# kxhit/semantic-icp

Hardware: AMD Instinct MI355X
Metric: correspondences/sec (higher is better)
Workload: dtype f64

## Files before the change

### semantic-icp_amd/csrc/engine.hpp

```cpp
#ifndef SICP_ENGINE_HPP_
#define SICP_ENGINE_HPP_

#include <hip/hip_runtime.h>

#include <algorithm>
#include <array>
#include <atomic>
#include <chrono>
#include <condition_variable>
#include <cmath>
#include <cstdio>
#include <cstdlib>
#include <cstring>
#include <deque>
#include <limits>
#include <memory>
#include <mutex>
#include <new>
#include <string>
#include <thread>
#include <unordered_map>
#include <unordered_set>
#include <vector>

// ... 249 lines not shown
  DevBuf<double> proj;
  bool proj_valid = false;
  DevBuf<int> nn;
  int nn_stride = 0;
  bool feat_valid = false;
  int feat_k = 0, feat_C = 0, feat_float_products = 0;
  bool feat_hist = false;
  unsigned long long feat_epoch = 0;
  unsigned long long proj_cm_id = 0;
  OwnedEvent ready_ev;
  std::atomic<bool> pending{false};
  int n_seg() const { return (int)seg_label.size(); }
  int caller_index(int d) const { return keep.empty() ? perm[d] : keep[perm[d]]; }
};

constexpr int kPoolDevices = 64;
constexpr size_t kPoolCap = 1024;
struct CloudPool {
  std::mutex m;
  std::vector<Cloud*> free_list[kPoolDevices];
};
CloudPool& cloud_pool();
std::shared_ptr<Cloud> acquire_cloud(int device);
unsigned long long next_epoch();
double now_ms();
bool debug_enabled();

struct JobSlice {
  int knn_K = 0;
  std::vector<sicp::KnnArgs> knn;
  std::vector<sicp::CovArgs> cov;
  std::vector<sicp::ProjArgs> proj;
  std::vector<sicp::WeightArgs> weight;
  std::vector<sicp::CountJob> count;
  struct Sizes { size_t knn = 0, cov = 0, proj = 0, weight = 0, count = 0; };
  Sizes sizes() const { return {knn.size(), cov.size(), proj.size(), weight.size(), count.size()}; }
  void shrink_to(const Sizes& s) { knn.resize(s.knn); cov.resize(s.cov); proj.resize(s.proj); weight.resize(s.weight); count.resize(s.count); }
  void clear() { shrink_to(Sizes()); }
  bool empty() const { return knn.empty() && cov.empty() && proj.empty() && weight.empty() && count.empty(); }
};

constexpr int kParts = 4;

struct JobCollector {
  bool fold_weights = false;
  int slice = 0;
  JobSlice part[kParts];
};

struct TickSet {
  DevBuf<sicp::BatchArgs> d_batch;
  DevBuf<sicp::BatchHeader> d_bhdr;
  HostBuf<sicp::BatchHeader> h_bhdr;
  HostBuf<sicp::BatchArgs> h_batch;
  HostBuf<sicp::LmJoin> h_join;
  DevBuf<sicp::LmJoin> d_join;
  int cap = 0;
  sicp::BatchGraph graph[2];
  bool static_ranges = false;
  std::vector<int> tick_act;
  bool tick_valid = false;
  TickSet() = default;
  TickSet(const TickSet&) = delete;
  TickSet& operator=(const TickSet&) = delete;
  ~TickSet() { sicp::batch_graph_destroy(graph[0]); sicp::batch_graph_destroy(graph[1]); }
  void invalidate() { tick_valid = false; tick_act.clear(); static_ranges = false; }
};

}
}

using namespace sicp::host;

struct sicp_use_state {
  JobCollector* collect = nullptr;
  sicp_params params;
  unsigned long long epoch = 0;
  int C = 0;
  std::vector<double> cm;
  unsigned long long cm_id = 0;
  int corr_n = 0, corr_K = 0;
  bool corr_valid = false, corr_weighted = false;
  bool hint_ok = false;
  int solo_pair = 0;
  bool solo_was_init = false, solo_failed = false;
  int solo_skip = 0, solo_penalty = 0;
  bool count_stats = false;
  bool counted_in_search = false;
  bool wait_on_device = false;
  std::string last_error;
  sicp_stats st = {};
  sicp_use_state() { sicp_default_params(SICP_MODE_GICP, &params); }
};

struct sicp_context : sicp_use_state {
  int device = 0;
  bool parked = false;
  std::shared_ptr<Cloud> cl[2];
  Cloud& cloud(int which) { return *cl[which]; }
  const Cloud& cloud(int which) const { return *cl[which]; }
  OwnedStream own_stream, own_stream2;
  OwnedStream side_stream;
  OwnedStream feat_stream;
  OwnedStream part_stream[kParts];
  JobSlice own_jobs;
  hipStream_t stream = nullptr, stream2 = nullptr;
  OwnedEvent ev0, ev1, ev_join;
  OwnedEvent side_done, side_done2, main_done;
  std::vector<OwnedEvent> chunk_ev;
  OwnedEvent part_fork, part_done[kParts];
  DevBuf<double> d_cm, d_hval;
  int hval_k = 0;
  DevBuf<int> idx;
  DevBuf<float> d2;
  DevBuf<double> w;
  DevBuf<unsigned long long> part;
  DevBuf<double> partials, out28;
  DevBuf<long long> d_count;
  DevBuf<sicp::LmState> d_lm;
  HostBuf<sicp::LmState> h_lm;
  HostBuf<double> h_out28;
  HostBuf<long long> h_count;
  DevBuf<float> tmpx, tmpy, tmpz;
  DevBuf<double> tmp9;
  DevBuf<uint32_t> tmpl;
  HostBuf<uint32_t> h_labels;
  HostBuf<unsigned char> pc_stage;
  DevBuf<int> ev_idx;
  DevBuf<float> ev_d2;
  HostBuf<unsigned char> ev_stage;
  HostBuf<unsigned char> mg_stage;
  HostBuf<uint32_t> mg_out;
  TickSet ts[2];
  DevBuf<sicp::LmState> d_bstates;
  DevBuf<double> d_bout28;
  HostBuf<sicp::LmState> h_bstates{hipHostMallocCoherent};
  HostBuf<double> h_bout28;
  DevBuf<unsigned> d_solo_sync;
  unsigned solo_tag = 0;
  int solo_seq = 0;
  HostBuf<int> h_solo_flag{hipHostMallocCoherent};

  void reset_use() {
    static_cast<sicp_use_state&>(*this) = sicp_use_state();
    stream = own_stream;
    stream2 = own_stream2;
    for (TickSet& S : ts) S.invalidate();
  }
};

struct StreamCloudRef;
namespace sicp {
namespace host {
struct PoseCovSums {
  double out28[28];
  double sums[42];
  long long active;
};
struct PoseCovStream;
}
}
struct sicp_stream_ctx {
  int device = 0, cap = 0;
  sicp_params params;
  int C = 0;
  std::vector<double> cm;
// ... 426 lines not shown
```

### semantic-icp_amd/csrc/kernels.h

```cpp
#ifndef SICP_KERNELS_H_
#define SICP_KERNELS_H_

#include <hip/hip_runtime.h>
#include <stdint.h>

#include "bvh.hpp"
#include "lm.hpp"

#ifndef SICP_HD
#define SICP_HD
#endif

namespace sicp {

struct Pose {
  double R[9];
  double t[3];
};

struct Mat4f {
  float m[16];
};

struct alignas(16) PointRec {
// ... 3 lines not shown
  float z;
  uint32_t pad_[3];
};
static_assert(sizeof(PointRec) == 48, "PointRec is read with three dwordx4 / dwordx2 loads");

#ifndef SICP_SG4
#define SICP_SG4 4
#endif
#ifndef SICP_ACC_OCC
#define SICP_ACC_OCC 2
#endif
constexpr int acc_slots_per_group(int K) { return K % 4 == 0 ? SICP_SG4 : 2; }

struct AccGeometry {
  int n_groups, steps, chunk_groups, n_chunks;
};
SICP_HD inline AccGeometry acc_geometry(int total_slots, int slots_per_group) {
  AccGeometry g;
  const int per_lane = 8 / slots_per_group;
  g.n_groups = (total_slots + slots_per_group - 1) / slots_per_group;
  int m = (g.n_groups + 256 * per_lane * 1024 - 1) / (256 * per_lane * 1024);
  if (m < 1) m = 1;
  g.steps = per_lane * m;
  g.chunk_groups = 256 * g.steps;
  g.n_chunks = (g.n_groups + g.chunk_groups - 1) / g.chunk_groups;
  if (g.n_chunks < 1) g.n_chunks = 1;
  return g;
}

struct LossArgs {
  double cauchy_a;
  int use_sqloss;
};

struct NNArgs {
  const float *qx, *qy, *qz;
  int q_begin, q_count;
  int do_xform;
  double M[12];
  const float4* pts4;
  int t_begin, t_count;
  int chunk_len;
  unsigned long long* part;
};

struct MergeArgs {
  int q_begin, q_count, n_chunks;
  const unsigned long long* part;
  const int* inv;
  float gate_sq;
  int* out_i;
  float* out_d;
  int k_out;
};

struct TreeArgs {
  const float4* pts4;
  const float4* box_lo;
  const float4* box_hi;
  const unsigned long long* leaf_code;
  TreeLevels lv;
  int n;
  int pt_begin;
  int node_begin;
  int code_begin;
  float lo[3];
  float scale;
};

struct KnnArgs {
  const float *qx, *qy, *qz;
  int q_begin, q_count;
  int do_xform;
  double M[12];
  TreeArgs tree;
  int self;
  float gate_sq;
  const int* inv;
  int* out_i;
  float* out_d;
  int* dbg;
  const int* seed_hint;
  int hint_K, t_begin;
  int out_stride;
  int k_out;
  unsigned long long* live_cnt;
  const PointRec *w_srec, *w_trec;
  const double *w_sproj, *w_tproj;
  double* w_out;
  double w_one_m_eps;
  int w_C, w_bool_probability;
};
constexpr int kLiveCounters = 1024;

struct CovArgs {
  int n, k, C;
  const float *x, *y, *z;
  const uint32_t* label;
  const int* nn;
  int nn_stride;
  int float_products;
  PointRec* rec;
  uint8_t* hist;
  char* rec_dense;
  int rec_dense_n;
};

SICP_HD inline size_t dense_rec_bytes(int n) { return (size_t)(n > 0 ? n : 1) * 36; }
constexpr int kDenseGatherMaxPoints = 1 << 27;

SICP_HD inline int hist_stride(int C) { return (C + 15) & ~15; }

SICP_HD inline int proj_stride(int C) { return (C + 1) & ~1; }

struct ProjArgs {
  int n, C;
  const uint8_t* hist;
  const double* cm;
  const double* hval;
  double* proj;
};

struct WeightArgs {
  int n_s, K, C;
  const int* idx;
  const PointRec *srec, *trec;
  const double *s_proj, *t_proj;
  const uint8_t *s_hist, *t_hist;
  const double *cm, *hval;
  Pose pose;
  double one_m_eps;
  int bool_probability;
  double* w;
};

struct AccArgs {
  int n_s, K;
  const int* idx;
  const double* w;
  const PointRec *srec, *trec;
  const char* srec_dense;
  const char* trec_dense;
  int n_t, pad_;
  Pose pose;
  const LmState* lm;
  LmState* lm_step;
  double one_m_eps;
  LossArgs loss;
  double* partials;
};

struct GenAccArgs {
  AccArgs a;
  const double *scov6, *tcov6;
  int n_chunks, pad_;
};
hipError_t launch_accumulate_general(const GenAccArgs& g, hipStream_t st);

constexpr int kMaxKnnJobs = 8;
constexpr int kMaxSmallJobs = 16;
struct KnnJobs { KnnArgs job[kMaxKnnJobs]; };
struct CovJobs { CovArgs job[kMaxSmallJobs]; };
struct ProjJobs { ProjArgs job[kMaxSmallJobs]; };
struct WeightJobs { WeightArgs job[kMaxKnnJobs]; };
struct CountJob { const int* idx; int n; unsigned long long* out; };
struct CountJobs { CountJob job[kMaxSmallJobs]; };
// ... 480 lines not shown
```

### semantic-icp_amd/csrc/knn_kernels.hip

```cpp
#include <hip/hip_runtime.h>
#include <stdint.h>
#include <stdlib.h>

#define SICP_HD __host__ __device__
#include "kernels.h"
#include "device_geometry.hpp"

namespace sicp {

__device__ __forceinline__ float xform_row(const double* m, double x, double y, double z) {
#pragma clang fp contract(off)
  double a = __dmul_rn(m[0], x);
  a = __dadd_rn(a, __dmul_rn(m[1], y));
  a = __dadd_rn(a, __dmul_rn(m[2], z));
  a = __dadd_rn(a, m[3]);
  return __double2float_rn(a);
}

__device__ __forceinline__ float l2_simple(float ax, float ay, float az, float bx, float by, float bz) {
#pragma clang fp contract(off)
  const float dx = __fsub_rn(ax, bx), dy = __fsub_rn(ay, by), dz = __fsub_rn(az, bz);
  float r = __fmul_rn(dx, dx);
  r = __fadd_rn(r, __fmul_rn(dy, dy));
  r = __fadd_rn(r, __fmul_rn(dz, dz));
// ... 181 lines not shown
}

template <int K, int Q, int BS, int TILE>
__global__ __launch_bounds__(BS) void nn_partial_kernel(NNArgs a) {
  __shared__ float4 tile[TILE];
  const int chunk = blockIdx.y;
  const int c_lo = chunk * a.chunk_len;
  const int c_hi = min(c_lo + a.chunk_len, a.t_count);

  float px[Q], py[Q], pz[Q], wd[Q];
  u64 bk[Q][K];
#pragma unroll
  for (int j = 0; j < Q; ++j) {
    int q = blockIdx.x * (BS * Q) + j * BS + threadIdx.x;
    q = min(q, a.q_count - 1);
    load_query(a.qx, a.qy, a.qz, a.q_begin + q, a.do_xform, a.M, px[j], py[j], pz[j]);
#pragma unroll
    for (int k = 0; k < K; ++k) bk[j][k] = KEY_EMPTY;
    wd[j] = key_dist(KEY_EMPTY);
  }

  for (int t0 = c_lo; t0 < c_hi; t0 += TILE) {
    const int n = min(TILE, c_hi - t0);
    __syncthreads();
    for (int p = threadIdx.x; p < n; p += BS) tile[p] = a.pts4[a.t_begin + t0 + p];
    __syncthreads();
#pragma unroll 4
    for (int p = 0; p < n; ++p) {
      const float4 t = tile[p];
#pragma unroll
      for (int j = 0; j < Q; ++j) consider<K>(bk[j], wd[j], l2_simple(px[j], py[j], pz[j], t.x, t.y, t.z), __float_as_uint(t.w));
    }
  }

#pragma unroll
  for (int j = 0; j < Q; ++j) {
    const int q = blockIdx.x * (BS * Q) + j * BS + threadIdx.x;
    if (q < a.q_count) {
      const size_t o = ((size_t)chunk * a.q_count + q) * K;
#pragma unroll
      for (int k = 0; k < K; ++k) a.part[o + k] = bk[j][k];
    }
  }
}

template <int K>
__global__ __launch_bounds__(256) void nn_merge_kernel(MergeArgs a) {
  const int q = blockIdx.x * blockDim.x + threadIdx.x;
  if (q >= a.q_count) return;
  u64 bk[K];
#pragma unroll
  for (int k = 0; k < K; ++k) bk[k] = KEY_EMPTY;
  for (int c = 0; c < a.n_chunks; ++c) {
    const size_t o = ((size_t)c * a.q_count + q) * K;
#pragma unroll
    for (int k = 0; k < K; ++k) {
      const u64 key = a.part[o + k];
      if (key < bk[K - 1]) key_insert<K>(bk, key);
    }
  }
  emit<K>(bk, a.inv, a.gate_sq, a.out_i, a.out_d, (size_t)(a.q_begin + q) * a.k_out, a.k_out);
}

__device__ __forceinline__ float box_lb(const float4 lo, const float4 hi, float px, float py, float pz) {
  const float ex = fmaxf(fmaxf(lo.x - px, px - hi.x), 0.f);
  const float ey = fmaxf(fmaxf(lo.y - py, py - hi.y), 0.f);
  const float ez = fmaxf(fmaxf(lo.z - pz, pz - hi.z), 0.f);
  return (ex * ex + ey * ey) + ez * ez;
}

__device__ __forceinline__ unsigned quad_min_u(unsigned v) {
  v = min(v, (unsigned)__builtin_amdgcn_mov_dpp((int)v, 0xB1, 0xf, 0xf, true));
  return min(v, (unsigned)__builtin_amdgcn_mov_dpp((int)v, 0x4E, 0xf, 0xf, true));
}
__device__ __forceinline__ unsigned quad_max_u(unsigned v) {
  v = max(v, (unsigned)__builtin_amdgcn_mov_dpp((int)v, 0xB1, 0xf, 0xf, true));
  return max(v, (unsigned)__builtin_amdgcn_mov_dpp((int)v, 0x4E, 0xf, 0xf, true));
}
template <int K>
__device__ __forceinline__ float quad_bound(const u64 (&bk)[K]) {
  constexpr int M = (K + 3) / 4;
  return __uint_as_float(min(quad_min_u((unsigned)(bk[K - 1] >> 32)), quad_max_u((unsigned)(bk[M - 1] >> 32))));
}

__device__ __forceinline__ void scan_points_quad4(const float4 (&t)[4], float px, float py, float pz, u64 (&bk)[4], float& wd) {
  u64 c[4];
  const knn_v2f qxy = {px, py};
#pragma unroll
  for (int p = 0; p < 4; ++p) c[p] = make_key(l2_simple_pk(qxy, pz, t[p].x, t[p].y, t[p].z), __float_as_uint(t[p].w));
  key_cswap(c[0], c[1]); key_cswap(c[2], c[3]); key_cswap(c[0], c[2]); key_cswap(c[1], c[3]); key_cswap(c[1], c[2]);
  double l[4];
#pragma unroll
  for (int i = 0; i < 4; ++i) {
    const double a = __longlong_as_double((long long)bk[i]), b = __longlong_as_double((long long)c[3 - i]);
    asm("v_min_f64 %0, %1, %2" : "=v"(l[i]) : "v"(a), "v"(b));
  }
#pragma unroll
  for (int i = 0; i < 4; ++i) bk[i] = (u64)__double_as_longlong(l[i]);
  key_cswap(bk[0], bk[2]); key_cswap(bk[1], bk[3]); key_cswap(bk[0], bk[1]); key_cswap(bk[2], bk[3]);
  wd = quad_bound<4>(bk);
}

template <int K>
__device__ __forceinline__ void scan_points_quad(const float4 (&t)[4], float px, float py, float pz, u64 (&bk)[K], float& wd) {
  if constexpr (K == 4) { scan_points_quad4(t, px, py, pz, bk, wd); return; }
  if constexpr (K >= 8) {
    u64 c[4];
    const knn_v2f qxy = {px, py};
#pragma unroll
    for (int p = 0; p < 4; ++p) c[p] = make_key(l2_simple_pk(qxy, pz, t[p].x, t[p].y, t[p].z), __float_as_uint(t[p].w));
    key_cswap(c[0], c[1]); key_cswap(c[2], c[3]); key_cswap(c[0], c[2]); key_cswap(c[1], c[3]); key_cswap(c[1], c[2]);
#pragma unroll
    for (int r = 0; r < 4; ++r) {
      const bool pass = !(key_dist(c[r]) > wd) && c[r] < bk[K - 1];
      if (__ballot(pass) == 0) break;
      if (pass) key_insert<K>(bk, c[r]);
    }
  } else {
#pragma unroll
    for (int p = 0; p < 4; ++p) {
      const float d = l2_simple(px, py, pz, t[p].x, t[p].y, t[p].z);
      if (!(d > wd)) {
        const u64 key = make_key(d, __float_as_uint(t[p].w));
        if (key < bk[K - 1]) key_insert<K>(bk, key);
      }
    }
  }
  wd = quad_bound<K>(bk);
}

template <int K>
__device__ __forceinline__ void scan_leaf_quad(const float4* __restrict__ pts, float px, float py, float pz, u64 (&bk)[K], float& wd) {
  float4 t[4];
#pragma unroll
  for (int p = 0; p < 4; ++p) t[p] = pts[4 * p];
  scan_points_quad<K>(t, px, py, pz, bk, wd);
}

__device__ __forceinline__ unsigned child_mask_quad(const float4* __restrict__ blo, const float4* __restrict__ bhi, int child_off,
                                                    int child_cnt, int parent, int sub, int lane, float px, float py, float pz,
                                                    float wd) {
  const int c = parent * kFan + sub;
  const int node = child_off + min(c, child_cnt - 1);
  const float lb = box_lb(blo[node], bhi[node], px, py, pz);
  const bool ok = c < child_cnt && !(lb > wd);
  return (unsigned)(__ballot(ok) >> (lane & ~3)) & 15u;
}

template <int K>
__global__ __launch_bounds__(64) void bvh_knn_quad_kernel(KnnArgs a) {
  __shared__ int s_off[kMaxLevels], s_cnt[kMaxLevels];
  __shared__ u64 s_merge[16][4][K];
  if (threadIdx.x < kMaxLevels) { s_off[threadIdx.x] = a.tree.lv.off[threadIdx.x]; s_cnt[threadIdx.x] = a.tree.lv.cnt[threadIdx.x]; }
  __syncthreads();
  const int lane = threadIdx.x, sub = lane & 3, slot = lane >> 2;
  const int q_raw = blockIdx.x * 16 + slot;
  const int q = min(q_raw, a.q_count - 1);
  float px, py, pz;
  load_query(a.qx, a.qy, a.qz, a.q_begin + q, a.do_xform, a.M, px, py, pz);
  u64 bk[K];
  key_list_init<K>(bk);
  float wd = INFINITY;
  const float4* __restrict__ pts_all = a.tree.pts4 + a.tree.pt_begin;
  const float4* __restrict__ pts = pts_all + sub;
  const float4* __restrict__ blo = a.tree.box_lo + a.tree.node_begin;
  const float4* __restrict__ bhi = a.tree.box_hi + a.tree.node_begin;
  const int top = a.tree.lv.n_levels - 1;
  const int n_leaf = s_cnt[0];

  int seed = 0;
  if (top >= 1) {
    if (a.self) {
      seed = (q / kLeaf) / kFan;
    } else {
      const u64 qc = curve_code(px, py, pz, a.tree.lo[0], a.tree.lo[1], a.tree.lo[2], a.tree.scale);
      const u64* __restrict__ codes = a.tree.leaf_code + a.tree.code_begin;
      int lo_i = 0, hi_i = n_leaf - 1;
      while (lo_i < hi_i) {
        const int mid = (lo_i + hi_i + 1) >> 1;
        if (codes[mid] <= qc) lo_i = mid; else hi_i = mid - 1;
      }
      seed = lo_i / kFan;
    }
    const int l0 = seed * kFan, l1 = min(l0 + kFan, n_leaf);
    for (int l = l0; l < l1; ++l) scan_leaf_quad<K>(pts + (size_t)l * kLeaf, px, py, pz, bk, wd);
  } else {
    scan_leaf_quad<K>(pts, px, py, pz, bk, wd);
  }

  if (top >= 2) {
    unsigned masks = 0, masks_hi = 0;
    auto get = [&](int lv) -> unsigned { return lv < 8 ? (masks >> (4 * lv)) & 15u : (masks_hi >> (4 * (lv - 8))) & 15u; };
    auto put = [&](int lv, unsigned m) {
      if (lv < 8) masks = (masks & ~(15u << (4 * lv))) | (m << (4 * lv));
      else masks_hi = (masks_hi & ~(15u << (4 * (lv - 8)))) | (m << (4 * (lv - 8)));
    };
    int L = top - 1, base = 0;
    put(L, child_mask_quad(blo, bhi, s_off[L], s_cnt[L], 0, sub, lane, px, py, pz, wd));
    bool done = false;
    while (!done) {
      int leaf = -1;
      while (leaf < 0 && !done) {
        const unsigned m = get(L);
        if (m == 0) {
          if (L == top - 1) { done = true; break; }
          ++L;
          base = (base / kFan) & ~(kFan - 1);
          continue;
        }
        const int c = __ffs(m) - 1;
        put(L, m & (m - 1));
        const int node = base + c;
        if (L == 1 && node == seed) continue;
        if (L == 0) {
          leaf = node;
        } else {
          put(L - 1, child_mask_quad(blo, bhi, s_off[L - 1], s_cnt[L - 1], node, sub, lane, px, py, pz, wd));
          --L;
          base = node * kFan;
// ... 22 lines not shown
      const float d = best == KEY_EMPTY ? INFINITY : key_dist(best);
      const bool keep = orig != 0xffffffffu && d < a.gate_sq;
      a.out_i[o + k] = keep ? a.inv[orig] : -1;
      if (a.out_d) a.out_d[o + k] = d;
    }
  }
}

__device__ __forceinline__ int xcd_contiguous_block(int bid, int nblk) {
  const int q = nblk >> 3, r = nblk & 7;
  const int xcd = bid & 7, loc = bid >> 3;
  return xcd < r ? xcd * (q + 1) + loc : r * (q + 1) + (xcd - r) * q + loc;
}

__device__ __forceinline__ unsigned child_mask_packet(const float4* __restrict__ blo, const float4* __restrict__ bhi, int child_off,
                                                      int parent, int sub, float px, float py, float pz, float wd, float& lb) {
  const int node = child_off + parent * kFan + sub;
  lb = box_lb(blo[node], bhi[node], px, py, pz);
  const bool ok = !(lb > wd);
  u64 b = __ballot(ok);
  b |= b >> 32; b |= b >> 16; b |= b >> 8; b |= b >> 4;
  return (unsigned)b & 15u;
}

__device__ __forceinline__ int locate_leaf(const u64* __restrict__ codes, int top, u64 qc, int lane) {
  int lo = 0, shift = 2 * top;
  const int i = lane & 15;
  while (shift > 0) {
    const int s = shift >= 4 ? shift - 4 : 0;
    const bool probe = i >= 1 && i < (1 << (shift - s));
    const u64 c = probe ? codes[lo + (i << s)] : ~0ull;
    const u64 below = __ballot(probe && c <= qc) & 0xfffeull;
    lo += __popcll(below) << s;
    shift = s;
  }
  return lo;
}

constexpr int kWalkLevels = kMaxLevels - 1;

#ifndef SICP_KNN_DMA_MAXK
#define SICP_KNN_DMA_MAXK 4
#endif
#define KNN_LDS __attribute__((address_space(3)))
#define KNN_GLOBAL __attribute__((address_space(1)))
typedef float knn_v4f __attribute__((ext_vector_type(4)));
__device__ __forceinline__ void dma_leaf_group(const float4* __restrict__ pts_all, unsigned group, KNN_LDS knn_v4f* buf, int lane) {
  const float4* p = pts_all + (size_t)group * (kFan * kLeaf) + lane;
  __builtin_amdgcn_global_load_lds((const KNN_GLOBAL void*)p, (KNN_LDS void*)buf, 16, 0, 0);
}
__device__ __forceinline__ void lds_leaf_points(const KNN_LDS knn_v4f* buf, unsigned c, int sub, float4 (&t)[4]) {
#pragma unroll
  for (int p = 0; p < 4; ++p) {
    const knn_v4f v = buf[c * kLeaf + sub + 4 * p];
    t[p] = make_float4(v.x, v.y, v.z, v.w);
  }
}

template <int K, int WPB, bool LITERAL = false>
__device__ __forceinline__ void knn_packet_body(const KnnArgs& a, int wg, int n_wg) {
  constexpr size_t kWaveBytes = sizeof(float) * kWalkLevels * 64;
  __shared__ __attribute__((aligned(16))) unsigned char s_wave_all[WPB][kWaveBytes];
  constexpr bool kDma = K <= SICP_KNN_DMA_MAXK;
  __shared__ __attribute__((aligned(16))) float4 s_pts_all[kDma ? WPB : 1][kDma ? kFan * kLeaf : 1];
  KNN_LDS knn_v4f* const s_pts = (KNN_LDS knn_v4f*)s_pts_all[kDma ? (threadIdx.x >> 6) : 0];
  float (&s_lb)[kWalkLevels][64] = *reinterpret_cast<float (*)[kWalkLevels][64]>(s_wave_all[threadIdx.x >> 6]);
  const int lane = threadIdx.x & 63, sub = lane & 3, slot = lane >> 2;
  const int bid = xcd_contiguous_block(wg, n_wg) * WPB + (int)(threadIdx.x >> 6);
  if (bid * 16 >= a.q_count) return;
  const int q_raw = bid * 16 + slot;
  const int q = min(q_raw, a.q_count - 1);
  float px, py, pz;
  load_query(a.qx, a.qy, a.qz, a.q_begin + q, a.do_xform, a.M, px, py, pz);
  u64 bk[K];
  key_list_init<K>(bk);
  float wd = INFINITY;
  const float4* __restrict__ pts_all = a.tree.pts4 + a.tree.pt_begin;
  const float4* __restrict__ pts = pts_all + sub;
  const float4* __restrict__ blo = a.tree.box_lo + a.tree.node_begin;
  const float4* __restrict__ bhi = a.tree.box_hi + a.tree.node_begin;
  const int top = a.tree.lv.n_levels - 1;

  int n_box = 0, n_scan = 0;
  if (top == 0) {
    scan_leaf_quad<K>(pts, px, py, pz, bk, wd);
    ++n_scan;
  } else {
    int seed_leaf;
    if (a.self) {
      seed_leaf = bid;
    } else {
      int prev = -1;
      if (a.seed_hint) prev = __builtin_amdgcn_readlane(a.seed_hint[(size_t)(a.q_begin + q) * a.hint_K], 32);
      if (prev >= a.t_begin && prev < a.t_begin + a.tree.n) {
        seed_leaf = (prev - a.t_begin) / kLeaf;
      } else {
        const u64 qc_lane = curve_code_coarse<10>(px, py, pz, a.tree.lo[0], a.tree.lo[1], a.tree.lo[2], a.tree.scale);
        const u64 qc = ((u64)(unsigned)__builtin_amdgcn_readlane((int)(qc_lane >> 32), 32) << 32) |
                       (unsigned)__builtin_amdgcn_readlane((int)qc_lane, 32);
        seed_leaf = locate_leaf(a.tree.leaf_code + a.tree.code_begin, top, qc, lane);
      }
    }
    seed_leaf = __builtin_amdgcn_readfirstlane(seed_leaf);
    u64 masks = 0;
    float cur_lb = 0.f;
    constexpr int PB = 4;
    if constexpr (kDma) dma_leaf_group(pts_all, (unsigned)seed_leaf >> 2, s_pts, lane);
    for (int L0 = 0; L0 < top; L0 += PB) {
      float4 lo[PB], hi[PB];
#pragma unroll
      for (int i = 0; i < PB; ++i) {
        const int L = min(L0 + i, top - 1);
        const int node = level_offset(top, L) + (((seed_leaf >> (2 * L)) & ~3) + sub);
        lo[i] = blo[node];
        hi[i] = bhi[node];
      }
#pragma unroll
      for (int i = 0; i < PB; ++i) {
        const int L = L0 + i;
        if (L < top) {
          const float lb = box_lb(lo[i], hi[i], px, py, pz);
          s_lb[L][lane] = lb;
          if (L == 0) cur_lb = lb;
          u64 b = __ballot(lb < INFINITY);
          b |= b >> 32; b |= b >> 16; b |= b >> 8; b |= b >> 4;
          const unsigned m4 = ((unsigned)b & 15u) & ~(1u << ((seed_leaf >> (2 * L)) & 3));
          masks |= (u64)m4 << (4 * L);
          ++n_box;
        }
      }
    }
    if constexpr (K >= 16) {
      if constexpr (kDma) asm volatile("s_waitcnt vmcnt(0)" ::: "memory");
#pragma unroll
      for (int l = 0; l < kFan; ++l) {
        float4 t[4];
        if constexpr (kDma) {
          lds_leaf_points(s_pts, (unsigned)l, sub, t);
        } else {
#pragma unroll
          for (int p = 0; p < 4; ++p) t[p] = pts[(size_t)((seed_leaf & ~3) + l) * kLeaf + 4 * p];
        }
#pragma unroll
        for (int p = 0; p < 4; ++p) bk[4 * l + p] = make_key(l2_simple_pk(knn_v2f{px, py}, pz, t[p].x, t[p].y, t[p].z), __float_as_uint(t[p].w));
      }
      key_sort16<K>(bk);
      wd = quad_bound<K>(bk);
      masks &= ~15ull;
      n_scan += 4;
    } else {
      if constexpr (kDma) {
        asm volatile("s_waitcnt vmcnt(0)" ::: "memory");
        float4 t[4];
        lds_leaf_points(s_pts, (unsigned)seed_leaf & 3u, sub, t);
        scan_points_quad<K>(t, px, py, pz, bk, wd);
      } else {
        scan_leaf_quad<K>(pts + (size_t)seed_leaf * kLeaf, px, py, pz, bk, wd);
      }
      ++n_scan;
    }
    unsigned sh = 0u, ubase = (unsigned)seed_leaf & ~3u;
    const unsigned t4 = 1u << (2 * (top + 1));
    auto drop_unneeded = [&]() {
      u64 b = __ballot(!(cur_lb > wd));
      b |= b >> 32; b |= b >> 16; b |= b >> 8; b |= b >> 4;
      masks &= ~((u64)(~(unsigned)b & 15u) << sh);
    };
    drop_unneeded();
    for (;;) {
      int leaf = -1;
      for (;;) {
        const u64 rest = masks >> sh;
        if (rest == 0) break;
        const unsigned m = (unsigned)rest & 15u;
        if (m == 0) {
          const unsigned up = (unsigned)__builtin_ctzll(rest) & ~3u;
          sh += up;
          ubase = (ubase >> (up >> 1)) & ~3u;
          cur_lb = s_lb[sh >> 2][lane];
          drop_unneeded();
          continue;
        }
        const unsigned c = (unsigned)__ffs(m) - 1u;
        masks ^= 1ull << (sh + c);
        const unsigned node = ubase + c;
        if (sh == 0u) { leaf = (int)node; break; }
        ++n_box;
        sh -= 4u;
        ubase = node * kFan;
        if constexpr (kDma)
          if (sh == 0u) dma_leaf_group(pts_all, node, s_pts, lane);
        const unsigned cm = child_mask_packet(blo, bhi, (int)((t4 - (t4 >> (sh >> 1))) / 3u), (int)node, sub, px, py, pz, wd, cur_lb);
        masks |= (u64)cm << sh;
        s_lb[sh >> 2][lane] = cur_lb;
      }
      if (leaf < 0) break;
      if constexpr (kDma) {
        asm volatile("s_waitcnt vmcnt(0)" ::: "memory");
        float4 t[4];
        lds_leaf_points(s_pts, (unsigned)leaf & 3u, sub, t);
        scan_points_quad<K>(t, px, py, pz, bk, wd);
      } else {
        scan_leaf_quad<K>(pts + (size_t)leaf * kLeaf, px, py, pz, bk, wd);
      }
      ++n_scan;
      drop_unneeded();
    }
  }
  if (a.dbg && sub == 0 && q_raw < a.q_count) { a.dbg[2 * q] = n_box; a.dbg[2 * q + 1] = n_scan; }

  quad_merge<K>(bk);
  {
    const size_t o = a.out_stride > 0 ? (size_t)(a.q_begin + q) : (size_t)(a.q_begin + q) * a.k_out;
    const size_t ks = a.out_stride > 0 ? (size_t)a.out_stride : 1;
    unsigned live = 0;
#pragma unroll
    for (int t = 0; t < (K + 3) / 4; ++t) {
      u64 best = bk[4 * t < K ? 4 * t : K - 1];
#pragma unroll
      for (int s2 = 1; s2 < 4; ++s2)
        if (4 * t + s2 < K) best = sub == s2 ? bk[4 * t + s2] : best;
      const int k = 4 * t + sub;
      const bool mine = q_raw < a.q_count && k < K && k < a.k_out;
      const unsigned orig = (unsigned)best;
      const float d = best == KEY_EMPTY ? INFINITY : key_dist(best);
      const bool keep = orig != 0xffffffffu && d < a.gate_sq;
      int nb = -1;
      if (mine) {
        if (keep) nb = a.inv[orig];
        a.out_i[o + k * ks] = nb;
        if (a.out_d) a.out_d[o + k * ks] = d;
      }
      if (a.live_cnt) live += (unsigned)__popcll(__ballot(mine && keep));
      if constexpr (K == 4) {
        if (a.w_out != nullptr) {
          double w = 0.0;
          if (mine && nb >= 0) {
            const int C = a.w_C, PS = proj_stride(C), NP = PS / 2;
            typedef double v2d_t __attribute__((ext_vector_type(2)));
            const v2d_t* __restrict__ psrc = reinterpret_cast<const v2d_t*>(a.w_sproj + (size_t)(a.q_begin + q) * PS);
            const v2d_t* __restrict__ ptgt = reinterpret_cast<const v2d_t*>(a.w_tproj + (size_t)nb * PS);
            const PointRec sr = a.w_srec[a.q_begin + q], tr = a.w_trec[nb];
            double prob = 0.0;
            for (int kk = 0; kk < NP; ++kk) {
              const v2d_t tv = ptgt[kk], sv = psrc[kk];
              { double temp = tv.x; temp *= sv.x; prob += temp; }
              if (2 * kk + 1 < C) { double temp = tv.y; temp *= sv.y; prob += temp; }
            }
            Pose P;
#pragma unroll
            for (int r = 0; r < 3; ++r) {
              P.R[3 * r + 0] = a.M[4 * r + 0]; P.R[3 * r + 1] = a.M[4 * r + 1]; P.R[3 * r + 2] = a.M[4 * r + 2];
              P.t[r] = a.M[4 * r + 3];
            }
            w = prob * slot_gate<LITERAL>(P, a.w_one_m_eps, sr, tr, a.w_bool_probability);
          }
          if (mine) a.w_out[o + k * ks] = w;
        }
      }
    }
    if (a.live_cnt && lane == 0 && live) atomicAdd(a.live_cnt + (bid & (kLiveCounters - 1)), (unsigned long long)live);
  }
}

template <int K, int WPB, bool LITERAL = false>
__global__ __launch_bounds__(64 * WPB) void bvh_knn_packet_kernel(KnnArgs a) {
  knn_packet_body<K, WPB, LITERAL>(a, (int)blockIdx.x, (int)gridDim.x);
}

#ifndef SICP_KNN20_WAVES
#define SICP_KNN20_WAVES 1
#endif
template <int K, int WPB, bool LITERAL = false>
__global__ __launch_bounds__(64 * WPB, (K >= 16 ? SICP_KNN20_WAVES : 1)) void bvh_knn_packet_jobs_kernel(KnnJobs jobs) {
  const KnnArgs& a = jobs.job[blockIdx.y];
  const int n_wg = ((a.q_count + 15) / 16 + WPB - 1) / WPB;
  if ((int)blockIdx.x >= n_wg) return;
  knn_packet_body<K, WPB, LITERAL>(a, (int)blockIdx.x, n_wg);
}


static constexpr int NN_BS = 256;
static constexpr int NN_TILE = 1024;

int nn_queries_per_thread(int K) { return K == 1 ? 4 : (K <= 4 ? 2 : 1); }

// ... 86 lines not shown
```

### semantic-icp_amd/csrc/stages.cpp

```cpp
#include "engine.hpp"

namespace sicp {
namespace host {

static int launch_slice(sicp_context* h, JobSlice& s, hipStream_t st) {
  if (!s.knn.empty()) HIPCHECK(sicp::launch_bvh_knn_packet_jobs(s.knn_K, s.knn.data(), (int)s.knn.size(), st));
  if (!s.cov.empty()) HIPCHECK(sicp::launch_cov_jobs(s.cov.data(), (int)s.cov.size(), st));
  if (!s.proj.empty()) HIPCHECK(sicp::launch_proj_jobs(s.proj.data(), (int)s.proj.size(), st));
  if (!s.weight.empty()) HIPCHECK(sicp::launch_em_weight_jobs(s.weight.data(), (int)s.weight.size(), st));
  if (!s.count.empty()) HIPCHECK(sicp::launch_count_active_jobs(s.count.data(), (int)s.count.size(), st));
  s.clear();
  return SICP_OK;
}

struct OwnLaunch {
  bool launched = false;
  double ms = 0.0;
};
template <class Add>
static int hand_off(sicp_context* h, hipStream_t stream, int timer_bit, Add add, OwnLaunch* own = nullptr) {
  if (h->collect) return add(h->collect->part[h->collect->slice]);
  JobSlice& one = h->own_jobs;
  one.clear();
  SICPCHECK(add(one));
  KernelTimer kt(h, stream == h->stream ? timer_bit : 0);
  if (!one.knn.empty() && one.knn_K > 1) {
    HIPCHECK(sicp::launch_bvh_knn_packet(one.knn_K, one.knn[0], stream));
    one.knn.clear();
  }
  SICPCHECK(launch_slice(h, one, stream));
  if (own) { own->launched = true; own->ms = kt.stop(); }
  return SICP_OK;
}

int run_nn(sicp_context* h, int K, const Cloud& Qc, int q_begin, int q_count, const double* M34, const Cloud& Tc,
           int tseg, bool self, float gate_sq, int* out_i, float* out_d, int timer_bit, hipStream_t stream, int out_stride,
           const WeightFold* fold) {
  if (q_count <= 0) return SICP_OK;
  const int L = sicp::nn_list_len(K);
  if (L == 0) return SICP_ERR_INVALID_ARGUMENT;
  const Cloud::SegTree& tr = Tc.trees[tseg];
  auto account = [&](double ms) {
    if (timer_bit == SICP_PROFILE_NN) { h->st.nn_kernel_ms += ms; h->st.nn_launches += 1; }
    else { h->st.cov_kernel_ms += ms; h->st.cov_launches += 1; }
  };
  if (h->params.nn_method >= 1) {
    sicp::KnnArgs a;
    a.qx = Qc.x.p; a.qy = Qc.y.p; a.qz = Qc.z.p;
    a.q_begin = q_begin; a.q_count = q_count;
    a.do_xform = M34 ? 1 : 0;
    for (int i = 0; i < 12; ++i) a.M[i] = M34 ? M34[i] : 0.0;
    a.tree.pts4 = Tc.pts4.p; a.tree.box_lo = Tc.box_lo.p; a.tree.box_hi = Tc.box_hi.p; a.tree.leaf_code = Tc.leaf_code.p;
    a.tree.lv = tr.lv; a.tree.n = tr.n; a.tree.pt_begin = tr.pt_begin; a.tree.node_begin = tr.node_begin;
    a.tree.code_begin = tr.code_begin;
    a.tree.lo[0] = tr.lo[0]; a.tree.lo[1] = tr.lo[1]; a.tree.lo[2] = tr.lo[2]; a.tree.scale = tr.scale;
    a.self = self ? 1 : 0;
    a.gate_sq = gate_sq;
    a.inv = Tc.inv.p;
    a.out_i = out_i; a.out_d = out_d;
    a.dbg = nullptr;
    a.out_stride = out_stride;
    a.k_out = K;
    a.live_cnt = nullptr;
    a.w_srec = a.w_trec = nullptr; a.w_sproj = a.w_tproj = nullptr; a.w_out = nullptr;
    a.w_one_m_eps = 0.0; a.w_C = 0; a.w_bool_probability = 0;
    if (fold && h->params.nn_method == 1) {
      a.w_srec = fold->srec; a.w_trec = fold->trec; a.w_sproj = fold->sproj; a.w_tproj = fold->tproj; a.w_out = fold->w;
      a.w_one_m_eps = fold->one_m_eps; a.w_C = fold->C; a.w_bool_probability = fold->bool_probability;
    }
    a.seed_hint = (!self && h->hint_ok && out_i == h->idx.p && h->corr_K == K && h->corr_n == Qc.n) ? h->idx.p : nullptr;
    a.hint_K = K;
    a.t_begin = Tc.seg_off.empty() ? 0 : Tc.seg_off[tseg];
    static const bool want_dbg = debug_enabled() && std::getenv("SICP_KNN_STATS") != nullptr;
    DevBuf<int> dbg;
    if (want_dbg) { HIPCHECK(dbg.reserve((size_t)2 * q_count)); a.dbg = dbg.p; }
    if (h->count_stats && !self && out_i == h->idx.p && h->params.nn_method == 1) {
      a.live_cnt = (unsigned long long*)h->d_count.p;
      h->counted_in_search = true;
    }
    OwnLaunch own;
    if (h->params.nn_method == 2) {
      KernelTimer kt(h, stream == h->stream ? timer_bit : 0);
      HIPCHECK(sicp::launch_bvh_knn_quad(L, a, stream));
      own.launched = true;
      own.ms = kt.stop();
    } else {
      SICPCHECK(hand_off(h, stream, timer_bit, [&](JobSlice& js) -> int {
        if (!js.knn.empty() && js.knn_K != L) {
          h->last_error = "internal: searches of two list lengths collected into one slice";
          return SICP_ERR_INVALID_ARGUMENT;
        }
        js.knn_K = L;
        js.knn.push_back(a);
        return SICP_OK;
      }, &own));
    }
    if (!own.launched) return SICP_OK;
    account(own.ms);
    if (want_dbg) {
      std::vector<int> hd((size_t)2 * q_count);
      HIPCHECK(hipMemcpy(hd.data(), dbg.p, sizeof(int) * hd.size(), hipMemcpyDeviceToHost));
      double sn = 0, sl = 0; int mn = 0, ml = 0;
      for (int i = 0; i < q_count; ++i) { sn += hd[2 * i]; sl += hd[2 * i + 1]; mn = std::max(mn, hd[2 * i]); ml = std::max(ml, hd[2 * i + 1]); }
      double wsum_n = 0, wsum_l = 0; int nw = 0;
      for (int w0 = 0; w0 < q_count; w0 += 64, ++nw) {
        int wn = 0, wl = 0;
        for (int i = w0; i < std::min(q_count, w0 + 64); ++i) { wn = std::max(wn, hd[2 * i]); wl = std::max(wl, hd[2 * i + 1]); }
        wsum_n += wn; wsum_l += wl;
      }
      std::fprintf(stderr, "[sicp knn stats] K=%d self=%d n=%d: boxes/query avg %.1f max %d (wave-max avg %.1f), leaves/query avg %.1f max %d (wave-max avg %.1f)\n",
                   K, (int)self, q_count, sn / q_count, mn, wsum_n / nw, sl / q_count, ml, wsum_l / nw);
      std::vector<int> pb, pl;
      for (int i = 0; i < q_count; i += 16) { pb.push_back(hd[2 * i]); pl.push_back(hd[2 * i + 1]); }
      std::sort(pb.begin(), pb.end()); std::sort(pl.begin(), pl.end());
      auto pct = [](const std::vector<int>& v, double f) { return v[std::min(v.size() - 1, (size_t)(f * v.size()))]; };
      std::fprintf(stderr, "[sicp knn stats]   per packet: boxes p50 %d p90 %d p99 %d p99.9 %d max %d | leaves p50 %d p90 %d p99 %d p99.9 %d max %d\n",
                   pct(pb, .5), pct(pb, .9), pct(pb, .99), pct(pb, .999), pb.back(), pct(pl, .5), pct(pl, .9), pct(pl, .99), pct(pl, .999), pl.back());
    }
    return SICP_OK;
  }
  const int t_count = tr.n;
  const int Q = sicp::nn_queries_per_thread(L);
  const int qblocks = (q_count + 256 * Q - 1) / (256 * Q);
  int chunks = (2048 + qblocks - 1) / qblocks;
  const int max_chunks = (t_count + 1023) / 1024;
  if (chunks > max_chunks) chunks = max_chunks;
  if (chunks < 1) chunks = 1;
  int chunk_len = (t_count + chunks - 1) / chunks;
  chunk_len = ((chunk_len + 1023) / 1024) * 1024;
  if (chunk_len < 1024) chunk_len = 1024;
  chunks = t_count > 0 ? (t_count + chunk_len - 1) / chunk_len : 1;
  const size_t need = (size_t)chunks * q_count * L;
  HIPCHECK(h->part.reserve(need));
  sicp::NNArgs a;
  a.qx = Qc.x.p; a.qy = Qc.y.p; a.qz = Qc.z.p;
  a.q_begin = q_begin; a.q_count = q_count;
  a.do_xform = M34 ? 1 : 0;
  for (int i = 0; i < 12; ++i) a.M[i] = M34 ? M34[i] : 0.0;
  a.pts4 = Tc.pts4.p;
  a.t_begin = tr.pt_begin; a.t_count = t_count;
  a.chunk_len = chunk_len;
  a.part = h->part.p;
  sicp::MergeArgs m;
  m.q_begin = q_begin; m.q_count = q_count; m.n_chunks = chunks;
  m.part = h->part.p;
  m.inv = Tc.inv.p;
  m.gate_sq = gate_sq;
  m.out_i = out_i; m.out_d = out_d;
  m.k_out = K;
  {
    KernelTimer kt(h, stream == h->stream ? timer_bit : 0);
    HIPCHECK(sicp::launch_nn_partial(L, a, chunks, stream));
    account(kt.stop());
  }
  HIPCHECK(sicp::launch_nn_merge(L, m, stream));
// ... 89 lines not shown
  if (!sicp::nn_k_supported(P.knn) || sicp::nn_list_len(P.k_cov) == 0) return SICP_ERR_INVALID_ARGUMENT;
  if (P.mode != SICP_MODE_GICP && (!h->cloud(0).has_label || !h->cloud(1).has_label)) return SICP_ERR_NOT_READY;
  if (P.mode == SICP_MODE_EM || need_cm) {
    if (P.num_classes < 1 || P.num_classes > 255 || h->C != P.num_classes) return SICP_ERR_NOT_READY;
    for (int wch = 0; wch < 2; ++wch) {
      const Cloud& c = h->cloud(wch);
      if (c.n > 0 && (c.label_min < 1 || c.label_max > (uint32_t)P.num_classes)) return SICP_ERR_BAD_LABEL;
    }
  }
  if (P.mode != SICP_MODE_SEMANTIC && h->cloud(1).n < P.knn) return SICP_ERR_TOO_FEW_POINTS;
  return SICP_OK;
}

void fill_pose(const double* qt, sicp::Pose& p) {
  sicp::se3::rotation(qt, p.R);
  p.t[0] = qt[4]; p.t[1] = qt[5]; p.t[2] = qt[6];
}

int segment_of(const Cloud& c, uint32_t label) {
  for (int k = 0; k < c.n_seg(); ++k)
    if (c.seg_label[k] == label) return k;
  return -1;
}

int count_active(sicp_context* h);
int run_weights(sicp_context* h, const double* qt);

int run_correspondences(sicp_context* h, const double* qt, int K, bool weights) {
  const sicp_params& P = h->params;
  Cloud &S = h->cloud(0), &T = h->cloud(1);
  const size_t slots = (size_t)(S.n > 0 ? S.n : 1) * K;
  HIPCHECK(h->idx.reserve(slots));
  HIPCHECK(h->d2.reserve(slots));
  HIPCHECK(h->w.reserve(slots));
  double M[12];
  matrix34(qt, M);
  const bool sem = P.mode == SICP_MODE_SEMANTIC;
  h->counted_in_search = false;
  WeightFold fold_args;
  const WeightFold* fold = nullptr;
  {
    const unsigned long long want_id = h->cm_id * 1099511628211ull + (unsigned long long)P.k_cov;
    bool ok = weights && P.mode == SICP_MODE_EM && K == 4 && P.nn_method == 1 && P.profile == 0 &&
              P.num_classes >= 1 && P.num_classes <= 16 && !weights_from_histograms(P, K) && S.n_seg() == 1 &&
              S.proj_valid && T.proj_valid && S.proj_cm_id == want_id && T.proj_cm_id == want_id;
    if (ok && h->collect) {
      ok = h->collect->fold_weights;
      for (const JobSlice& js : h->collect->part) ok = ok && js.cov.empty() && js.proj.empty();
    }
    if (ok) {
      fold_args.srec = S.rec.p; fold_args.trec = T.rec.p;
      fold_args.sproj = S.proj.p; fold_args.tproj = T.proj.p;
      fold_args.w = h->w.p;
      fold_args.one_m_eps = 1.0 - P.epsilon;
      fold_args.C = P.num_classes;
      fold_args.bool_probability = P.quirk_bool_probability;
      fold = &fold_args;
    }
  }
  if (sem) {
    HIPCHECK(hipMemsetAsync(h->idx.p, 0xFF, sizeof(int) * slots, h->stream));
    HIPCHECK(hipMemsetD32Async((hipDeviceptr_t)h->d2.p, 0x7f800000, slots, h->stream));
  }
  {
    const double t0 = now_ms();
    for (int s = 0; s < S.n_seg(); ++s) {
      const int so = S.seg_off[s], sn = S.seg_off[s + 1] - so;
      int ts = 0;
      if (sem) {
        ts = segment_of(T, S.seg_label[s]);
        if (ts < 0) continue;
        if (!(sn > P.min_class_pts)) continue;
      }
      SICPCHECK(run_nn(h, K, S, so, sn, M, T, ts, false, (float)P.gate_sq, h->idx.p, h->d2.p, SICP_PROFILE_NN, h->stream, 0, fold));
      h->st.total_corr += (int64_t)sn * K;
    }
    h->st.t_nn_ms += now_ms() - t0;
  }
  h->corr_weighted = false;
  h->corr_n = S.n;
  h->corr_K = K;
  h->corr_valid = true;
  h->hint_ok = true;
  if (h->count_stats && !h->counted_in_search) SICPCHECK(count_active(h));
  if (weights && fold) {
    h->corr_weighted = true;
    ++h->st.weights_in_search;
  } else if (weights) {
    SICPCHECK(run_weights(h, qt));
  }
  return SICP_OK;
}

int search_at(sicp_context* h, const double* qt) {
  const sicp_params& P = h->params;
  const bool em = P.mode == SICP_MODE_EM;
  Cloud &S = h->cloud(0), &T = h->cloud(1);
  SICPCHECK(prepare_cloud(h, S));
  SICPCHECK(prepare_cloud(h, T));
  if (!features_current(h, S, em)) SICPCHECK(compute_features(h, S, em));
  if (!features_current(h, T, em)) SICPCHECK(compute_features(h, T, em));
  if (em && !weights_from_histograms(P, P.knn)) {
    SICPCHECK(ensure_proj(h, S));
    SICPCHECK(ensure_proj(h, T));
  }
  return run_correspondences(h, qt, P.knn, true);
}

bool weights_from_histograms(const sicp_params& P, int K) {
  static const bool on = std::getenv("SICP_WEIGHTS_FROM_HIST") != nullptr;
  return on && P.mode == SICP_MODE_EM && K == 4 && P.num_classes >= 1 && P.num_classes <= 16;
}

int run_weights(sicp_context* h, const double* qt) {
  const sicp_params& P = h->params;
  Cloud &S = h->cloud(0), &T = h->cloud(1);
  const int K = h->corr_K;
  if (P.mode == SICP_MODE_EM) {
    const double t0 = now_ms();
    sicp::WeightArgs a{};
    a.n_s = S.n; a.K = K; a.C = P.num_classes;
    a.idx = h->idx.p;
    a.srec = S.rec.p; a.trec = T.rec.p;
    if (weights_from_histograms(P, K)) {
      SICPCHECK(ensure_hval(h, P.k_cov));
      a.s_hist = S.hist.p; a.t_hist = T.hist.p;
      a.cm = h->d_cm.p; a.hval = h->d_hval.p;
    } else {
      SICPCHECK(ensure_proj(h, S));
      SICPCHECK(ensure_proj(h, T));
      a.s_proj = S.proj.p; a.t_proj = T.proj.p;
    }
    fill_pose(qt, a.pose);
    a.one_m_eps = 1.0 - P.epsilon;
    a.bool_probability = P.quirk_bool_probability;
    a.w = h->w.p;
    OwnLaunch own;
    SICPCHECK(hand_off(h, h->stream, SICP_PROFILE_WEIGHT, [&](JobSlice& js) -> int { js.weight.push_back(a); return SICP_OK; }, &own));
    h->st.weight_launches += 1;
    h->st.weight_kernel_ms += own.ms;
    h->st.t_weight_ms += now_ms() - t0;
    h->corr_weighted = true;
  }
  return SICP_OK;
}

void fill_acc(sicp_context* h, sicp::AccArgs& a) {
  const sicp_params& P = h->params;
  Cloud &S = h->cloud(0), &T = h->cloud(1);
  a.n_s = h->corr_n; a.K = h->corr_K;
  a.idx = h->idx.p;
  a.w = h->corr_weighted ? h->w.p : nullptr;
  a.srec = S.rec.p; a.trec = T.rec.p;
  a.srec_dense = (S.rec_dense_n == S.n && S.n > 0 && S.n == h->corr_n) ? S.rec_dense.p : nullptr;
  a.trec_dense = (T.feat_valid && T.rec_dense_n == T.n && T.n > 0 && T.n <= sicp::kDenseGatherMaxPoints) ? T.rec_dense.p : nullptr;
  a.n_t = T.n; a.pad_ = 0;
  a.lm = nullptr;
  a.lm_step = nullptr;
  a.one_m_eps = 1.0 - P.epsilon;
  a.loss.cauchy_a = P.cauchy_a;
  a.loss.use_sqloss = P.use_sqloss;
  a.partials = h->partials.p;
}

bool general_covariances(const sicp_context* h) { return h->cloud(0).cov_general || h->cloud(1).cov_general; }

// ... 177 lines not shown
```

Baseline: 2.635 billion.

## Use previous-iteration neighbors as KNN distance bound and gate seed reuse by pose motion

For small K, the quad BVH KNN kernel now loads the previous iteration's neighbor point for each lane and uses its distance as an initial pruning bound. This tightens the search radius from the start so fewer boxes and leaves get visited. The host also records the pose used for the hint. It passes the pose delta and a motion threshold so the kernel stops trusting the old seed leaf when the query has moved far. This adds extra loads and arithmetic per query, and a wrong bound could change results if the hint point is not a valid candidate.

```diff
diff --git a/semantic-icp_amd/csrc/engine.hpp b/semantic-icp_amd/csrc/engine.hpp
--- a/semantic-icp_amd/csrc/engine.hpp
+++ b/semantic-icp_amd/csrc/engine.hpp
@@ -355,6 +355,7 @@
   int corr_n = 0, corr_K = 0;
   bool corr_valid = false, corr_weighted = false;
   bool hint_ok = false;
+  double hint_M[12] = {};
   int solo_pair = 0;
   bool solo_was_init = false, solo_failed = false;
   int solo_skip = 0, solo_penalty = 0;
diff --git a/semantic-icp_amd/csrc/kernels.h b/semantic-icp_amd/csrc/kernels.h
--- a/semantic-icp_amd/csrc/kernels.h
+++ b/semantic-icp_amd/csrc/kernels.h
@@ -109,6 +109,8 @@
   int* dbg;
   const int* seed_hint;
   int hint_K, t_begin;
+  float hint_dM[12];
+  float seed_move_sq;
   int out_stride;
   int k_out;
   unsigned long long* live_cnt;
diff --git a/semantic-icp_amd/csrc/knn_kernels.hip b/semantic-icp_amd/csrc/knn_kernels.hip
--- a/semantic-icp_amd/csrc/knn_kernels.hip
+++ b/semantic-icp_amd/csrc/knn_kernels.hip
@@ -287,8 +287,16 @@
   constexpr int M = (K + 3) / 4;
   return __uint_as_float(min(quad_min_u((unsigned)(bk[K - 1] >> 32)), quad_max_u((unsigned)(bk[M - 1] >> 32))));
 }
-
-__device__ __forceinline__ void scan_points_quad4(const float4 (&t)[4], float px, float py, float pz, u64 (&bk)[4], float& wd) {
+constexpr unsigned kNoHintBound = (unsigned)(0x7fefffffffffffffull >> 32);
+template <int K, bool HINT>
+__device__ __forceinline__ float quad_bound(const u64 (&bk)[K], unsigned hint) {
+  if constexpr (!HINT) return quad_bound<K>(bk);
+  constexpr int M = (K + 3) / 4;
+  return __uint_as_float(min(min(quad_min_u((unsigned)(bk[K - 1] >> 32)), quad_max_u((unsigned)(bk[M - 1] >> 32))), hint));
+}
+
+template <bool HINT>
+__device__ __forceinline__ void scan_points_quad4(const float4 (&t)[4], float px, float py, float pz, u64 (&bk)[4], float& wd, unsigned hint) {
   u64 c[4];
   const knn_v2f qxy = {px, py};
 #pragma unroll
@@ -303,12 +311,13 @@
 #pragma unroll
   for (int i = 0; i < 4; ++i) bk[i] = (u64)__double_as_longlong(l[i]);
   key_cswap(bk[0], bk[2]); key_cswap(bk[1], bk[3]); key_cswap(bk[0], bk[1]); key_cswap(bk[2], bk[3]);
-  wd = quad_bound<4>(bk);
-}
-
-template <int K>
-__device__ __forceinline__ void scan_points_quad(const float4 (&t)[4], float px, float py, float pz, u64 (&bk)[K], float& wd) {
-  if constexpr (K == 4) { scan_points_quad4(t, px, py, pz, bk, wd); return; }
+  wd = quad_bound<4, HINT>(bk, hint);
+}
+
+template <int K, bool HINT = false>
+__device__ __forceinline__ void scan_points_quad(const float4 (&t)[4], float px, float py, float pz, u64 (&bk)[K], float& wd,
+                                                 unsigned hint = kNoHintBound) {
+  if constexpr (K == 4) { scan_points_quad4<HINT>(t, px, py, pz, bk, wd, hint); return; }
   if constexpr (K >= 8) {
     u64 c[4];
     const knn_v2f qxy = {px, py};
@@ -331,15 +340,16 @@
       }
     }
   }
-  wd = quad_bound<K>(bk);
-}
-
-template <int K>
-__device__ __forceinline__ void scan_leaf_quad(const float4* __restrict__ pts, float px, float py, float pz, u64 (&bk)[K], float& wd) {
+  wd = quad_bound<K, HINT>(bk, hint);
+}
+
+template <int K, bool HINT = false>
+__device__ __forceinline__ void scan_leaf_quad(const float4* __restrict__ pts, float px, float py, float pz, u64 (&bk)[K], float& wd,
+                                               unsigned hint = kNoHintBound) {
   float4 t[4];
 #pragma unroll
   for (int p = 0; p < 4; ++p) t[p] = pts[4 * p];
-  scan_points_quad<K>(t, px, py, pz, bk, wd);
+  scan_points_quad<K, HINT>(t, px, py, pz, bk, wd, hint);
 }
 
 __device__ __forceinline__ unsigned child_mask_quad(const float4* __restrict__ blo, const float4* __restrict__ bhi, int child_off,
@@ -528,17 +538,40 @@
   const int top = a.tree.lv.n_levels - 1;
 
   int n_box = 0, n_scan = 0;
+  constexpr bool kHintBound = K <= 4;
+  unsigned hint_bound = kNoHintBound;
   if (top == 0) {
     scan_leaf_quad<K>(pts, px, py, pz, bk, wd);
     ++n_scan;
   } else {
     int seed_leaf;
+    float4 hp = make_float4(0.f, 0.f, 0.f, 0.f);
+    bool hint_in = false;
     if (a.self) {
       seed_leaf = bid;
     } else {
       int prev = -1;
-      if (a.seed_hint) prev = __builtin_amdgcn_readlane(a.seed_hint[(size_t)(a.q_begin + q) * a.hint_K], 32);
-      if (prev >= a.t_begin && prev < a.t_begin + a.tree.n) {
+      bool moved_far = false;
+      if (a.seed_hint) {
+        const bool bound_wanted = kHintBound && a.hint_K >= K;
+        const int entry = K == 1 || !bound_wanted ? 0 : sub;
+        const int prev_lane = a.seed_hint[(size_t)(a.q_begin + q) * a.hint_K + entry];
+        {
+          const float x = a.qx[a.q_begin + q], y = a.qy[a.q_begin + q], z = a.qz[a.q_begin + q];
+          const float* d = a.hint_dM;
+          const float mx = fmaf(d[0], x, fmaf(d[1], y, fmaf(d[2], z, d[3])));
+          const float my = fmaf(d[4], x, fmaf(d[5], y, fmaf(d[6], z, d[7])));
+          const float mz = fmaf(d[8], x, fmaf(d[9], y, fmaf(d[10], z, d[11])));
+          const float m2 = fmaf(mx, mx, fmaf(my, my, mz * mz));
+          moved_far = __uint_as_float((unsigned)__builtin_amdgcn_readlane((int)__float_as_uint(m2), 32)) > a.seed_move_sq;
+        }
+        prev = __builtin_amdgcn_readlane(prev_lane, 32);
+        if constexpr (kHintBound) {
+          hint_in = bound_wanted && prev_lane >= a.t_begin && prev_lane < a.t_begin + a.tree.n;
+          hp = pts_all[hint_in ? prev_lane - a.t_begin : 0];
+        }
+      }
+      if (!moved_far && prev >= a.t_begin && prev < a.t_begin + a.tree.n) {
         seed_leaf = (prev - a.t_begin) / kLeaf;
       } else {
         const u64 qc_lane = curve_code_coarse<10>(px, py, pz, a.tree.lo[0], a.tree.lo[1], a.tree.lo[2], a.tree.scale);
@@ -576,6 +609,11 @@
         }
       }
     }
+    if constexpr (kHintBound) {
+      const unsigned hb = hint_in ? __float_as_uint(l2_simple(px, py, pz, hp.x, hp.y, hp.z)) : kNoHintBound;
+      hint_bound = quad_max_u(hb);
+      wd = __uint_as_float(min(__float_as_uint(wd), hint_bound));
+    }
     if constexpr (K >= 16) {
       if constexpr (kDma) asm volatile("s_waitcnt vmcnt(0)" ::: "memory");
 #pragma unroll
@@ -599,9 +637,9 @@
         asm volatile("s_waitcnt vmcnt(0)" ::: "memory");
         float4 t[4];
         lds_leaf_points(s_pts, (unsigned)seed_leaf & 3u, sub, t);
-        scan_points_quad<K>(t, px, py, pz, bk, wd);
+        scan_points_quad<K, kHintBound>(t, px, py, pz, bk, wd, hint_bound);
       } else {
-        scan_leaf_quad<K>(pts + (size_t)seed_leaf * kLeaf, px, py, pz, bk, wd);
+        scan_leaf_quad<K, kHintBound>(pts + (size_t)seed_leaf * kLeaf, px, py, pz, bk, wd, hint_bound);
       }
       ++n_scan;
     }
@@ -645,9 +683,9 @@
         asm volatile("s_waitcnt vmcnt(0)" ::: "memory");
         float4 t[4];
         lds_leaf_points(s_pts, (unsigned)leaf & 3u, sub, t);
-        scan_points_quad<K>(t, px, py, pz, bk, wd);
+        scan_points_quad<K, kHintBound>(t, px, py, pz, bk, wd, hint_bound);
       } else {
-        scan_leaf_quad<K>(pts + (size_t)leaf * kLeaf, px, py, pz, bk, wd);
+        scan_leaf_quad<K, kHintBound>(pts + (size_t)leaf * kLeaf, px, py, pz, bk, wd, hint_bound);
       }
       ++n_scan;
       drop_unneeded();
diff --git a/semantic-icp_amd/csrc/stages.cpp b/semantic-icp_amd/csrc/stages.cpp
--- a/semantic-icp_amd/csrc/stages.cpp
+++ b/semantic-icp_amd/csrc/stages.cpp
@@ -32,6 +32,11 @@
   if (own) { own->launched = true; own->ms = kt.stop(); }
   return SICP_OK;
 }
+
+#ifndef SICP_SEED_MOVE_LEAVES
+#define SICP_SEED_MOVE_LEAVES 0.25
+#endif
+static constexpr double kSeedMoveLeaves = SICP_SEED_MOVE_LEAVES;
 
 int run_nn(sicp_context* h, int K, const Cloud& Qc, int q_begin, int q_count, const double* M34, const Cloud& Tc,
            int tseg, bool self, float gate_sq, int* out_i, float* out_d, int timer_bit, hipStream_t stream, int out_stride,
@@ -71,6 +76,13 @@
     a.seed_hint = (!self && h->hint_ok && out_i == h->idx.p && h->corr_K == K && h->corr_n == Qc.n) ? h->idx.p : nullptr;
     a.hint_K = K;
     a.t_begin = Tc.seg_off.empty() ? 0 : Tc.seg_off[tseg];
+    for (int i = 0; i < 12; ++i) a.hint_dM[i] = a.seed_hint && M34 ? (float)(M34[i] - h->hint_M[i]) : 0.f;
+    {
+      const double ext = 2097151.0 / (double)tr.scale;
+      const double leaves = (double)std::max(1, (tr.n + sicp::kLeaf - 1) / sicp::kLeaf);
+      const double move = kSeedMoveLeaves * ext / std::sqrt(leaves);
+      a.seed_move_sq = (float)(move * move);
+    }
     static const bool want_dbg = debug_enabled() && std::getenv("SICP_KNN_STATS") != nullptr;
     DevBuf<int> dbg;
     if (want_dbg) { HIPCHECK(dbg.reserve((size_t)2 * q_count)); a.dbg = dbg.p; }
@@ -326,6 +338,7 @@
   h->corr_K = K;
   h->corr_valid = true;
   h->hint_ok = true;
+  std::memcpy(h->hint_M, M, sizeof h->hint_M);
   if (h->count_stats && !h->counted_in_search) SICPCHECK(count_active(h));
   if (weights && fold) {
     h->corr_weighted = true;
```

Result: no change. 2.658 billion (median of 6 runs) (+0.9%).
